# mehta-lab/VisCy

Measured on AMD Instinct MI355X. Metric: training patches/sec (Z=5, 256x256, 1->2ch UNeXt2), higher is better.
Workload: dtype bf16; 1 GPU; UNeXt2 2.5D convnextv2_tiny Z=5 256x256 1->2ch, fwd+MixedLoss(0.5,0,0.5)+bwd+AdamW; per_gpu_batch=512, global_batch=512, parallelism=dp1

## Files before the change

include/vsx.h:

```cpp
#ifndef VSX_H
#define VSX_H
#include <stddef.h>
#include <stdint.h>

#ifdef __cplusplus
extern "C" {
#endif

typedef void* vsx_stream_t;

#define VSX_F32 0
#define VSX_BF16 1

int32_t vsx_version(void);
const char* vsx_last_error(void);
const char* vsx_last_kernel(void);
int32_t vsx_set_flag(const char* name, int32_t value);
int32_t vsx_get_flag(const char* name);
int32_t vsx_det_workspace(float* ws, int64_t floats);
int32_t vsx_det_scope(int32_t on);
int32_t vsx_det_active(void);

#define VSX_A_ROWS 0
#define VSX_A_PATCH2 1
// ... 281 lines not shown
#define VSX_WTASK_REDUCE_ROWS 6
#define VSX_WTASK_MAX 40
typedef struct VsxWTask {
  int32_t kind, dtype, i0, i1, i2, i3;
  const void* p0;
  void* p1;
  void* p2;
  const void* p3;
  const void* p4;
  const void* p5;
  const void* p6;
  const void* p7;
} VsxWTask;
int32_t vsx_weight_tasks(const VsxWTask* tasks, int32_t n, vsx_stream_t stream);

int32_t vsx_prep_head_dgrad(const float* W, void* dst, int32_t Cmid, int32_t C3, int32_t Zout, int32_t dtype,
    vsx_stream_t stream);

int32_t vsx_stem_im2col(const float* x, void* P, const float* sub, const float* div, int32_t B, int32_t Cin,
    int32_t Z, int32_t H, int32_t W, int32_t kz, int32_t ky, int32_t kx, int32_t dtype, vsx_stream_t stream);
int32_t vsx_stem_im2col_ld(const float* x, void* P, const float* sub, const float* div, int32_t B, int32_t Cin, int32_t Z,
    int32_t H, int32_t W, int32_t kz, int32_t ky, int32_t kx, int32_t ldp, int32_t dtype, vsx_stream_t stream);
int32_t vsx_pad_cols(const void* src, void* dst, int32_t R, int32_t K, int32_t Kp, int32_t dtype, vsx_stream_t stream);

int32_t vsx_im2col3x3(const void* x, void* col, int32_t B, int32_t H, int32_t W, int32_t C, int32_t dtype, vsx_stream_t stream);
int32_t vsx_col2im3x3(const void* dcol, void* dx, int32_t B, int32_t H, int32_t W, int32_t C, int32_t dtype, vsx_stream_t stream);

int32_t vsx_pixel_shuffle_cat_fwd(const void* low, const void* skip, void* out, int32_t B, int32_t h,
    int32_t w, int32_t c, int32_t cs, int32_t dtype, vsx_stream_t stream);

int32_t vsx_pixel_shuffle_cat_bwd(const void* dcat, void* dlow, void* dskip, int32_t B, int32_t h, int32_t w,
    int32_t c, int32_t cs, int32_t dtype, vsx_stream_t stream);

int32_t vsx_head_shuffle_fwd(const void* dec, void* hin, int32_t B, int32_t h, int32_t w, int32_t C3,
    int32_t D, int32_t pool, int32_t dtype, vsx_stream_t stream);

int32_t vsx_head_shuffle_bwd(const void* dhin, void* ddec, int32_t B, int32_t h, int32_t w, int32_t C3,
    int32_t D, int32_t pool, int32_t dtype, vsx_stream_t stream);

int32_t vsx_normalize(const float* x, float* y, const float* sub, const float* div, int32_t B, int64_t per_sample,
    vsx_stream_t stream);

int32_t vsx_minmax_norm(const float* x, float* y, const float* lo, const float* hi, int32_t B, int64_t per_sample,
    vsx_stream_t stream);

int32_t vsx_sample_minmax(const float* x, float* mn, float* mx, int32_t B, int64_t per_sample, vsx_stream_t stream);

int32_t vsx_intensity_aug(const float* x, float* y, const float* mn, const float* mx, const float* gamma,
    const float* factor, const float* noise, const float* nstd, float nmean, int32_t invert, int32_t B, int64_t per_sample,
    vsx_stream_t stream);
int32_t vsx_sample_moments(const float* x, double* sums, int32_t B, int64_t per_sample, vsx_stream_t stream);

int32_t vsx_blend_in(const float* oldp, const float* newp, float* out, const float* fz, int32_t Z, int64_t plane,
    int64_t total, vsx_stream_t stream);

int32_t vsx_crop_weights(const float* w, float* wpool, float* tmp, int32_t B, int32_t CZ, int32_t Y, int32_t X,
    int32_t cy, int32_t cx, vsx_stream_t stream);
int32_t vsx_sample_index(const float* wpool, const float* u, int32_t* idx, int32_t B, int64_t n, vsx_stream_t stream);
int32_t vsx_crop3d(const float* x, float* y, const int32_t* starts, int32_t B, int32_t C, int32_t Z, int32_t Y, int32_t X,
    int32_t cz, int32_t cy, int32_t cx, vsx_stream_t stream);

int32_t vsx_warp_affine3d(const float* x, float* y, const float* Minv, int32_t B, int32_t C, int32_t D, int32_t H,
    int32_t W, int32_t mode, vsx_stream_t stream);
int32_t vsx_warp_affine3d_roi(const float* x, float* y, const float* Minv, int32_t B, int32_t C, int32_t D, int32_t H,
    int32_t W, int32_t z0, int32_t y0, int32_t x0, int32_t Do, int32_t Ho, int32_t Wo, int32_t mode, vsx_stream_t stream);

// ... 31 lines not shown
```

viscy_amd/_lib.py:

```python

from __future__ import annotations

import ctypes as C
import os

import torch

_HERE = os.path.dirname(os.path.abspath(__file__))
LIB_PATH = os.environ.get("VSX_LIB", os.path.join(_HERE, "libvsx.so"))

VSX_F32, VSX_BF16 = 0, 1
A_ROWS, A_PATCH2, A_CONV3 = 0, 1, 2
PRO_NONE, PRO_GRN = 0, 1
EPI_NONE, EPI_BIAS, EPI_BIAS_GELU_SQ, EPI_BIAS_RES, EPI_DZ, EPI_BIAS_STATS, EPI_LN_BWD = 0, 1, 2, 3, 4, 5, 6
LOSS_SLOTS, LOSS_SLOT_STRIDE = 64, 32

_I32, _F32, _P, _I64 = C.c_int32, C.c_float, C.c_void_p, C.c_int64


class VsxGemm(C.Structure):
    _fields_ = [
        ("A", _P), ("B", _P), ("C", _P),
        ("M", _I32), ("N", _I32), ("K", _I32),
        ("lda", _I32), ("ldb", _I32), ("ldc", _I32),
# ... 27 lines not shown


WTASK_PREP, WTASK_TRANSPOSE, WTASK_MATVEC, WTASK_MLP_PACK, WTASK_UNPREP, WTASK_MATVEC_T, WTASK_REDUCE_ROWS = 0, 1, 2, 3, 4, 5, 6

_SIGS = {
    "vsx_version": (_I32, []),
    "vsx_weight_tasks": (_I32, [_P, _I32, _P]),
    "vsx_last_error": (C.c_char_p, []),
    "vsx_last_kernel": (C.c_char_p, []),
    "vsx_set_flag": (_I32, [C.c_char_p, _I32]),
    "vsx_get_flag": (_I32, [C.c_char_p]),
    "vsx_det_workspace": (_I32, [_P, _I64]),
    "vsx_det_scope": (_I32, [_I32]),
    "vsx_det_active": (_I32, []),
    "vsx_gemm_nt": (_I32, [C.POINTER(VsxGemm), _I32, _P]),
    "vsx_gemm_tn": (_I32, [C.POINTER(VsxGemm), _I32, _P]),
    "vsx_gemm_plan": (_I32, [_I32, C.POINTER(VsxGemm), _I32, C.POINTER(VsxGemmPlan)]),
    "vsx_gemm_nt_ln_bwd_supported": (_I32, [_I64, _I32, _I32, _I32]),
    "vsx_ln_fwd": (_I32, [_P, _P, _P, _P, _P, _P, _I32, _I32, _F32, _I32, _P]),
    "vsx_ln_bwd": (_I32, [_P, _P, _P, _P, _P, _P, _P, _P, _P, _I32, _I32, _I32, _P]),
    "vsx_grn_scale": (_I32, [_P, _P, _P, _I32, _I32, _F32, _P]),
    "vsx_grn_bwd_stats": (_I32, [_P, _P, _P, _P, _P, _P, _P, _P, _I32, _I32, _F32, _P]),
    "vsx_grn_gelu_bwd": (_I32, [_P, _P, _P, _P, _P, _P, _I32, _I32, _I32, _I32, _I32, _P]),
    "vsx_dwconv7_fwd": (_I32, [_P, _P, _P, _P, _P, _I32, _I32, _I32, _I32, _I32, _P]),
    "vsx_dwconv7_bwd_data": (_I32, [_P, _P, _P, _P, _I32, _I32, _I32, _I32, _I32, _P]),
    "vsx_dwconv7_bwd_weight": (_I32, [_P, _P, _P, _P, _P, _I32, _I32, _I32, _I32, _I32, _I32, _P]),
    "vsx_stem_im2col": (_I32, [_P, _P, _P, _P, _I32, _I32, _I32, _I32, _I32, _I32, _I32, _I32, _I32, _P]),
    "vsx_stem_im2col_ld": (_I32, [_P, _P, _P, _P, _I32, _I32, _I32, _I32, _I32, _I32, _I32, _I32, _I32, _I32, _P]),
    "vsx_pad_cols": (_I32, [_P, _P, _I32, _I32, _I32, _I32, _P]),
    "vsx_im2col3x3": (_I32, [_P, _P, _I32, _I32, _I32, _I32, _I32, _P]),
    "vsx_col2im3x3": (_I32, [_P, _P, _I32, _I32, _I32, _I32, _I32, _P]),
    "vsx_pixel_shuffle_cat_fwd": (_I32, [_P, _P, _P, _I32, _I32, _I32, _I32, _I32, _I32, _P]),
    "vsx_pixel_shuffle_cat_bwd": (_I32, [_P, _P, _P, _I32, _I32, _I32, _I32, _I32, _I32, _P]),
    "vsx_head_shuffle_fwd": (_I32, [_P, _P, _I32, _I32, _I32, _I32, _I32, _I32, _I32, _P]),
    "vsx_head_shuffle_bwd": (_I32, [_P, _P, _I32, _I32, _I32, _I32, _I32, _I32, _I32, _P]),
    "vsx_head_out_fwd": (_I32, [_P] * 7 + [_I32] * 6 + [_F32, _I32, _P]),
    "vsx_head_out_bwd1": (_I32, [_P] * 11 + [_I32] * 6 + [_F32, _I32, _P]),
    "vsx_head_out_bwd1_wgrad": (_I32, [_P] * 13 + [_I32] * 6 + [_F32, _I32, _P]),
    "vsx_head_out_bwd2": (_I32, [_P] * 9 + [_I32] * 6 + [_F32, _I32, _P]),
    "vsx_loss_pool": (_I32, [_P] * 7 + [_I32] * 3 + [_P]),
    "vsx_ssim_scale_fwd": (_I32, [_P] * 5 + [_I32] * 5 + [_P]),
    "vsx_ssim_scale_bwd": (_I32, [_P] * 7 + [_I32] * 5 + [_F32, _F32, _P, _I32, _P]),
    "vsx_loss_finalize": (_I32, [_P] * 5 + [_F32, _I32, _I32, _I32, _F32, _F32, _F32, _P, _P, _P, _P, _P]),
    "vsx_ssim_scale_fwd_dmu": (_I32, [_P] * 6 + [_I32] * 6 + [_P]),
    "vsx_ssim_scale_bwd_in": (_I32, [_P] * 6 + [_I32] * 5 + [_F32, _F32, _P, _I32, _I32, _P]),
    "vsx_loss_tmax": (_I32, [_P, _I64, _P, _P]),
    "vsx_ssim_scale_fwd_fused": (_I32, [_P] * 11 + [_I32] * 6 + [_P]),
    "vsx_adamw": (_I32, [_P, _P, _P, _P, _P, _I64, _P]),
    "vsx_adamw_advance": (_I32, [_P, _P, _P, _P]),
    "vsx_fill_f32": (_I32, [_P, _I64, _F32, _P]),
    "vsx_mlp_supported": (_I32, [_I32, _I32, _I64, _I32]),
    "vsx_mlp_mode_supported": (_I32, [_I32, _I32, _I64, _I32, _I32]),
    "vsx_mlp_det_floats": (_I64, [_I32, _I32, _I64, _I32]),
    "vsx_mlp_image_bytes": (_I64, [_I32]),
    "vsx_mlp_pack": (_I32, [_P, _P, _P, _I32, _P]),
    "vsx_mlp_fwd": (_I32, [_P] * 11 + [_I64, _I32, _I32, _I32, _I32, _P]),
    "vsx_mlp_fc1": (_I32, [_P] * 7 + [_I64, _I32, _I32, _I32, _P]),
    "vsx_mlp_fwd_ln": (_I32, [_P, _F32] + [_P] * 10 + [_I64, _I32, _I32, _I32, _I32, _P]),
    "vsx_mlp_fc1_ln": (_I32, [_P, _F32] + [_P] * 9 + [_I64, _I32, _I32, _I32, _P]),
    "vsx_grn_q_reduce": (_I32, [_P] * 10 + [_I64, _I32, _I32, _I32, _P]),
    "vsx_grn_q_reduce_ws_floats": (_I64, [_I32, _I32]),
    "vsx_mlp_bwd_stats": (_I32, [_P] * 5 + [_I64, _I32, _I32, _I32, _P]),
    "vsx_mlp_bwd_dh": (_I32, [_P] * 7 + [_I64, _P, _P, _I64, _I32, _I32, _I32, _P]),
    "vsx_mlp_rows_per_workgroup": (_I32, [_I32, _I32, _I64]),
    "vsx_mlp_bwd_dh_re": (_I32, [_P] * 9 + [_I64, _P, _P, _I64, _I32, _I32, _I32, _P]),
    "vsx_mlp_bwd_dh_ln": (_I32, [_P] * 11 + [_I64, _P, _P, _I64, _I32, _I32, _I32, _P]),
# ... 124 lines not shown
```

viscy_amd/csrc/norm.hip:

```cpp
#include "vsx_common.h"
#include "wtasks.h"
#include "../../include/vsx.h"

template <typename T, int G, int CPL>
__global__ __launch_bounds__(256) void ln_fwd_kernel(const T* __restrict__ x, T* __restrict__ y,
                                                     float* __restrict__ mean_out, float* __restrict__ rstd_out,
                                                     const float* __restrict__ gamma, const float* __restrict__ beta,
                                                     int rows, int C, float eps, int iters, int nt) {
  constexpr int VN = VT<T>::N;
  constexpr int R = CPL == 1 ? 4 : (CPL == 2 ? 2 : 1);
  constexpr int RPI = 256 / G;
  const int nch = C / VN;
  const int gl = threadIdx.x % G;
  float gam[CPL][VN], bet[CPL][VN];
#pragma unroll
  for (int i = 0; i < CPL; ++i) {
    const int c = gl + i * G;
#pragma unroll
    for (int j = 0; j < VN; ++j) {
      gam[i][j] = (gamma && c < nch) ? gamma[c * VN + j] : 1.f;
      bet[i][j] = (gamma && c < nch) ? beta[c * VN + j] : 0.f;
    }
  }
  for (int it = 0; it < iters; ++it) {
// ... 235 lines not shown
  if (nch <= 192) LN_CASE(64, 3);
  if (nch <= 256) LN_CASE(64, 4);
#undef LN_CASE
  vsx_set_error("layernorm: C=%d too wide (max %d)", C, 256 * VT<T>::N);
  return 1;
}

extern "C" int32_t vsx_ln_fwd(const void* x, void* y, float* mean, float* rstd, const float* gamma, const float* beta,
                              int32_t rows, int32_t C, float eps, int32_t dtype, vsx_stream_t stream) {
  int vn = dtype == VSX_BF16 ? 8 : 4;
  VSX_CHECK(rows > 0 && C > 0 && C % vn == 0, "vsx_ln_fwd: rows=%d C=%d (C must be a multiple of %d)", rows, C, vn);
  VSX_CHECK(x && y && rstd, "vsx_ln_fwd: null pointer");
  VSX_CHECK((gamma == nullptr) == (beta == nullptr), "vsx_ln_fwd: gamma and beta must both be set or both NULL");
  hipStream_t s = (hipStream_t)stream;
  return dtype == VSX_BF16
             ? ln_dispatch<bf16_t>(true, x, nullptr, y, mean, rstd, gamma, beta, nullptr, nullptr, nullptr, rows, C, eps, s)
             : ln_dispatch<float>(true, x, nullptr, y, mean, rstd, gamma, beta, nullptr, nullptr, nullptr, rows, C, eps, s);
}

extern "C" int32_t vsx_ln_bwd(const void* dy, const void* x, const float* mean, const float* rstd, const float* gamma,
                              const void* add, void* dx, float* dgamma, float* dbeta, int32_t rows, int32_t C,
                              int32_t dtype, vsx_stream_t stream) {
  int vn = dtype == VSX_BF16 ? 8 : 4;
  VSX_CHECK(rows > 0 && C > 0 && C % vn == 0, "vsx_ln_bwd: rows=%d C=%d (C must be a multiple of %d)", rows, C, vn);
  VSX_CHECK(dy && x && rstd && dx, "vsx_ln_bwd: null pointer");
  VSX_CHECK((dgamma == nullptr) == (dbeta == nullptr), "vsx_ln_bwd: dgamma and dbeta must both be set or both NULL");
  hipStream_t s = (hipStream_t)stream;
  return dtype == VSX_BF16 ? ln_dispatch<bf16_t>(false, dy, x, dx, (float*)mean, (float*)rstd, gamma, nullptr, add,
                                                 dgamma, dbeta, rows, C, 0.f, s)
                           : ln_dispatch<float>(false, dy, x, dx, (float*)mean, (float*)rstd, gamma, nullptr, add,
                                                dgamma, dbeta, rows, C, 0.f, s);
}

__global__ __launch_bounds__(256) void grn_scale_kernel(const float* __restrict__ colsq, const float* __restrict__ gamma,
                                                        float* __restrict__ s, int N, float eps) {
  __shared__ float part[4];
  const int b = blockIdx.x;
  float acc = 0.f;
  for (int n = threadIdx.x; n < N; n += 256) acc += sqrtf(colsq[(size_t)b * N + n]);
  acc = wave_sum(acc);
  if ((threadIdx.x & 63) == 0) part[threadIdx.x >> 6] = acc;
  __syncthreads();
  const float m = (part[0] + part[1] + part[2] + part[3]) / (float)N;
  for (int n = threadIdx.x; n < N; n += 256)
    s[(size_t)b * N + n] = 1.f + gamma[n] * sqrtf(colsq[(size_t)b * N + n]) / (m + eps);
}

__global__ __launch_bounds__(256) void grn_bwd_stats_kernel(const float* __restrict__ colsq, const float* __restrict__ P,
                                                            const float* __restrict__ gamma, float* __restrict__ t,
                                                            float* __restrict__ wsg, int N, float eps) {
  __shared__ float part[2][4];
  const int b = blockIdx.x;
  float a0 = 0.f, a1 = 0.f;
  for (int n = threadIdx.x; n < N; n += 256) {
    float g = sqrtf(colsq[(size_t)b * N + n]);
    a0 += g;
    a1 += gamma[n] * P[(size_t)b * N + n] * g;
  }
  a0 = wave_sum(a0);
  a1 = wave_sum(a1);
  if ((threadIdx.x & 63) == 0) { part[0][threadIdx.x >> 6] = a0; part[1][threadIdx.x >> 6] = a1; }
  __syncthreads();
  const float m = (part[0][0] + part[0][1] + part[0][2] + part[0][3]) / (float)N;
  const float sdg = part[1][0] + part[1][1] + part[1][2] + part[1][3];
  const float inv = 1.f / (m + eps);
  for (int n = threadIdx.x; n < N; n += 256) {
// ... 278 lines not shown
```

viscy_amd/engine_unext2.py:

```python

from __future__ import annotations

import os
from collections import namedtuple
from typing import NamedTuple

import torch
from torch import Tensor

from . import _lib as L
from . import ops as hip_ops
from .flat import FlatEngine, engine_apply


class _BlockW:

    __slots__ = ("C", "p", "dw_w", "W1f", "W1fT", "b1f", "W2", "W2T", "v1", "fc2_w", "fc2_b", "grn_w", "grn_b", "dp", "img", "img2", "b2f")


class _ProjW:
    __slots__ = ("cin", "cout", "taps", "ln", "conv", "W", "WT")


FWD_UNFUSED, FWD_PAIR, FWD_FC1 = 0, 1, 2
# ... 250 lines not shown
            W["fc0"], W["fc0T"] = o.prep_weight(t.fc0.weight, E, Cf, 1, torch.float32, want=True, want_t=need_bwd)
            W["fc3"], W["fc3T"] = o.prep_weight(t.fc3.weight, P, E, 1, torch.float32, want=True, want_t=need_bwd)
        else:
            for us in m.decoder.decoder_stages:
                st = us.conv
                proj = self._prep_proj(st.downsample[0], st.downsample[1], dt, need_bwd)
                dec.append((proj, [self._prep_block(b, dt, need_bwd) for b in st.blocks]))
            pre = []
            for us in m.decoder.decoder_stages:
                pc = getattr(us, "pre_conv", None)
                if pc is None:
                    pre.append(None)
                else:
                    cpc = pc.weight.shape[0]
                    pre.append((pc, *o.prep_weight(pc.weight, cpc, cpc, 9, dt, want=True, want_t=need_bwd)))
            W["dec_pre"] = pre
        W["dec"] = dec
        if cfg.get("head", "conv") == "conv":
            hc = m.head.conv[0].conv
            cmid, c3 = hc.weight.shape[0], hc.weight.shape[1]
            hdt = self._head_dtype(dt)
            W["head_Wc"], _ = o.prep_weight(hc.weight, cmid, c3, 27, hdt, tapmode=1)
            if need_bwd:
                if hdt == torch.bfloat16 and c3 == 8 and cmid == 32 and cfg["out_stack_depth"] == 5:
                    o.flush()
                    W["head_Wp"] = o.head_conv_dgrad_prep(W["head_Wc"])
                W["head_Wd"] = o.prep_head_dgrad(hc.weight, cmid, c3, cfg["out_stack_depth"], hdt)
        return W

    def _head_dtype(self, dt: torch.dtype) -> torch.dtype:
        if dt == torch.bfloat16 and self.model.head.conv[0].conv.weight.shape[1] % 8:
            return torch.float32
        return dt

    def _plan(self, C, hw, M, B, dt, training: bool) -> _MlpPlan:
        o, flag = self.ops, self._mlp_flag
        ask = training and dt == torch.bfloat16 and flag != 0
        return _plan_mlp(flag, lambda mode: o.mlp_supported(C, hw, M, dt, mode), C, hw, M, B, dt, training,
                         ask and bool(L.lib().vsx_gemm_nt_ln_bwd_supported(M, C, 4 * C, L.dtype_code(dt))),
                         ask and o.tn_grn_stats_ok(M, C, 4 * C, hw, dt))

    def _block_fwd(self, x, w, B, H, Wd, dt, save, rows=None):
        if w.C < 16:
            return self._block_fwd_narrow(x, w, B, H, Wd, save, rows)
        o = self.ops
        C, M = w.C, B * H * Wd
        blk = w.p
        hw = H * Wd
        y = o.dwconv7_fwd(x, w.dw_w, blk.conv_dw.bias, B, H, Wd, C)
        xres = x
        if rows is not None:
            idx, inv, _, Lr = rows
            M, hw = B * Lr, Lr
            y = o.rows_select(y, idx, M, C)
            xres = o.rows_select(x, idx, M, C)
        plan = self._plan(C, hw, M, B, dt, save is not None)
        mean = rstd = None
        if plan.ln_in:
            xh = None
        else:
            xh, _, rstd = o.ln_fwd(y, None, None, M, C, 1e-6, need_mean=False)
            y = None
        colsq = self._za.take(B, 4 * C)
        dpm = None
        if w.dp > 0.0 and self.model.training:
            inj = self._dp_inject
# ... 225 lines not shown
                       a_mode=L.A_PATCH2, gh=ch, gw=cw, cs=cc, epi=L.EPI_BIAS, bias=proj.conv.bias)
                st_sv["proj"] = (cur, xn, mean, rstd)
                cur, cc = nxt, proj.cout
            rows = None
            if masks is not None:
                rows = masks[i]
                cur = o.rows_select(cur, rows[2], B * ch * cw, cc)
            for bw in blocks:
                cur = self._block_fwd(cur, bw, B, ch, cw, dt, st_sv["blocks"] if need_bwd else None, rows)
            feats.append((cur, ch, cw, cc))
            enc_sv.append(st_sv)
        if cfg.get("head") == "embed":
            out = self._embed_tail_fwd(feats[3], B, sv, bn_groups)
            if need_bwd:
                sv["enc"] = enc_sv
                sv["feat_dims"] = [(a, b_, c) for (_, a, b_, c) in feats]
            self._za_need[za_key] = za.used
            return out, sv
        dec_sv = []
        feat, fh, fw, fc = feats[3]
        for k, (proj, blocks) in enumerate(W["dec"]):
            skip, sh, sw_, sc = feats[2 - k]
            assert sh == 2 * fh and sw_ == 2 * fw
            c_up = fc // 4
            pre = W["dec_pre"][k]
            low_in = None
            if pre is not None:
                pc, Wp, _ = pre
                col = o.im2col3x3(feat, B, fh, fw, fc)
                low_in = feat
                feat = torch.empty((B * fh * fw, fc), dtype=dt, device=x.device)
                o.gemm("nt", col, Wp, feat, B * fh * fw, fc, 9 * fc, 9 * fc, 9 * fc, fc, dtype=dt, epi=L.EPI_BIAS, bias=pc.bias)
                del col
            cat = o.pixel_shuffle_cat_fwd(feat, skip, B, fh, fw, c_up, sc)
            fh, fw = sh, sw_
            Mk, ccat = B * fh * fw, c_up + sc
            if proj.cout < 16:
                cur, mean, rstd = o.narrow_proj_fwd(cat, proj.ln.weight, proj.ln.bias, proj.conv.weight, proj.conv.bias, Mk, ccat,
                                                    proj.cout)
                xn = None
            else:
                xn, mean, rstd = o.ln_fwd(cat, proj.ln.weight, proj.ln.bias, Mk, ccat)
                cur = torch.empty((Mk, proj.cout), dtype=dt, device=x.device)
                o.gemm("nt", xn, proj.W, cur, Mk, proj.cout, ccat, ccat, ccat, proj.cout, dtype=dt, epi=L.EPI_BIAS,
                       bias=proj.conv.bias)
            st_sv = {"proj": (cat, xn, mean, rstd, c_up, sc), "blocks": [], "pre_in": low_in}
            for bw in blocks:
                cur = self._block_fwd(cur, bw, B, fh, fw, dt, st_sv["blocks"] if need_bwd else None)
            feat, fc = cur, proj.cout
            dec_sv.append(st_sv)
        if cfg.get("head", "conv") == "shuffle":
            sxy = cfg["stem_kernel"][-1]
            out = o.voxel_shuffle_fwd(feat, B, fh, fw, cfg["out_channels"], cfg["out_stack_depth"], sxy, True)
            if need_bwd:
                sv["enc"], sv["dec"] = enc_sv, dec_sv
                sv["feat_dims"] = [(a, b_, c) for (_, a, b_, c) in feats]
                sv["head"] = (fh, fw)
            self._za_need[za_key] = za.used
            return out, sv
        Zo, D7 = cfg["out_stack_depth"], cfg["out_stack_depth"] + 2
        hc = m.head.conv[0].conv
        cmid, c3 = hc.weight.shape[0], hc.weight.shape[1]
        cout = cfg["out_channels"]
        hdt = self._head_dtype(dt)
        hin = o.head_shuffle_fwd(feat if hdt == dt else feat.float(), B, fh, fw, c3, D7, cfg["head_pool"])
        H2, W2 = 2 * fh, 2 * fw
        Mh = B * H2 * W2
        stats = self._za.take(2, B, cmid)
        direct = o.head_conv_supported(H2, W2, c3, cmid, Zo, hdt)
        if direct:
            U = o.head_conv_fwd(hin, W["head_Wc"], hc.bias, stats[0], stats[1], B, H2, W2, c3, cmid, Zo)
        else:
            U = torch.empty((Mh, Zo * cmid), dtype=hdt, device=x.device)
            o.gemm_z("nt", hin, W["head_Wc"], U, Mh, cmid, 27 * c3, D7 * c3, 27 * c3, Zo * cmid, dtype=hdt,
                     a_mode=L.A_CONV3, gh=H2, gw=W2, cs=3 * c3, nz=Zo, a_coff=[z * c3 for z in range(Zo)],
                     b_off=[0] * Zo, c_coff=[z * cmid for z in range(Zo)], epi=L.EPI_BIAS_STATS, bias=hc.bias,
                     red0=stats[0], red1=stats[1], hw=H2 * W2)
        w2 = m.head.conv[1].weight.view(4 * cout, cmid)
        out = o.head_out_fwd(U, stats[0], stats[1], w2, m.head.conv[1].bias, m.head.conv[0].adn.A.weight, B, H2, W2, Zo,
# ... 122 lines not shown
            za_key = ("bwd", B, H, Wd, sv["masked"])
            self._za = za = _ZeroArena(dev, self._za_need.get(za_key, 0), self.ops)
            if cfg.get("head") == "embed":
                d = self._embed_tail_bwd(sv, dout[0], dout[1], dt, B)
            elif cfg.get("head", "conv") == "shuffle":
                fh, fw = sv["head"]
                sxy = cfg["stem_kernel"][-1]
                vs = o.voxel_shuffle_bwd
                if (cfg["out_channels"] * cfg["out_stack_depth"] * sxy * sxy) % (8 if dt == torch.bfloat16 else 4):
                    vs = o.narrow_voxel_shuffle_bwd
                d = vs(dout.contiguous().float(), B, fh, fw, cfg["out_channels"], cfg["out_stack_depth"], sxy, True, dt)
            else:
                hdt = self._head_dtype(dt)
                d = self._head_conv_bwd(sv, dout, hdt, B, dev)
                if hdt != dt:
                    d = d.to(dt)
            dskips = {}
            for k in (2, 1, 0) if cfg.get("head") != "embed" else ():
                proj, blocks = W["dec"][k]
                st_sv = sv["dec"][k]
                cat, xn, mean, rstd, c_up, sc = st_sv["proj"]
                _, sh, sw_, _ = (None, *sv["feat_dims"][2 - k])
                Mk, ccat = B * sh * sw_, c_up + sc
                for bw, bsv in zip(reversed(blocks), reversed(st_sv["blocks"])):
                    d = self._block_bwd(d, bw, bsv, B, sh, sw_, dt)
                if proj.cout < 16:
                    dxn = o.narrow_proj_bwd(d, cat, mean, rstd, proj.ln.weight, proj.ln.bias, proj.conv.weight, g(proj.conv.weight),
                                            g(proj.conv.bias), Mk, ccat, proj.cout)
                else:
                    o.gemm("tn", xn, d, g(proj.conv.weight), Mk, proj.cout, ccat, ccat, proj.cout, ccat, dtype=dt,
                           colsum=g(proj.conv.bias))
                    dxn = torch.empty((Mk, ccat), dtype=dt, device=dev)
                    o.gemm("nt", d, proj.WT, dxn, Mk, ccat, proj.cout, proj.cout, proj.cout, ccat, dtype=dt)
                dcat = o.ln_bwd(dxn, cat, mean, rstd, proj.ln.weight, None, g(proj.ln.weight), g(proj.ln.bias), Mk, ccat)
                del dxn
                d, dskips[2 - k] = o.pixel_shuffle_cat_bwd(dcat, B, sh // 2, sw_ // 2, c_up, sc)
                del dcat
                pre = W["dec_pre"][k]
                if pre is not None:
                    pc, _, WpT = pre
                    lh, lw, cpc = sh // 2, sw_ // 2, 4 * c_up
                    Ml = B * lh * lw
                    col = o.im2col3x3(st_sv["pre_in"], B, lh, lw, cpc)
                    dWp = self._za.take(cpc, 9 * cpc)
                    o.gemm("tn", col, d, dWp, Ml, cpc, 9 * cpc, 9 * cpc, cpc, 9 * cpc, dtype=dt, colsum=g(pc.bias))
                    o.unprep_grad(dWp, g(pc.weight), cpc, cpc, 9)
                    del col
                    dcol = torch.empty((Ml, 9 * cpc), dtype=dt, device=dev)
                    o.gemm("nt", d, WpT, dcol, Ml, 9 * cpc, cpc, cpc, cpc, 9 * cpc, dtype=dt)
                    d = o.col2im3x3(dcol, B, lh, lw, cpc)
                    del dcol
            yield from self._segment_end(0)
            if self.encoder_frozen():
                self._za_need[za_key] = za.used
                yield from self._segment_end(1)
                yield from self._segment_end(2)
                return
            for i in (3, 2, 1, 0):
                proj, blocks = W["enc"][i]
                st_sv = sv["enc"][i]
                ch, cw, cc = sv["feat_dims"][i]
                for bw, bsv in zip(reversed(blocks), reversed(st_sv["blocks"])):
                    d = self._block_bwd(d, bw, bsv, B, ch, cw, dt)
                if proj is not None:
                    prev, xn, mean, rstd = st_sv["proj"]
                    cin = proj.cin
                    Mo = B * ch * cw
                    dWg = self._za.take(proj.cout, 4 * cin)
                    o.gemm("tn", xn, d, dWg, Mo, proj.cout, 4 * cin, cin, proj.cout, 4 * cin, dtype=dt, a_mode=L.A_PATCH2,
                           gh=ch, gw=cw, cs=cin, colsum=g(proj.conv.bias))
# ... 46 lines not shown
```

viscy_amd/ops.py:

```python

from __future__ import annotations

import contextlib
import ctypes as C
import os
import threading
from typing import Sequence

import torch
from torch import Tensor

from . import _lib as L
from ._lib import VsxGemm, VsxGemmPlan, check, dtype_code, lib, ptr, stream


class Scratch:

    def __init__(self, alloc=None):
        self._alloc = alloc or (lambda floats, dev: torch.empty(floats, dtype=torch.float32, device=dev))
        self._tls = threading.local()
        self.held: list = []

    def take(self, dev, floats: int):
        arenas = getattr(self._tls, "arenas", None)
# ... 229 lines not shown
    col = torch.empty((B * H * W, 9 * Cc), dtype=x.dtype, device=x.device)
    check(lib().vsx_im2col3x3(ptr(x), ptr(col), B, H, W, Cc, dtype_code(x.dtype), stream()), "im2col3x3")
    return col


def col2im3x3(dcol: Tensor, B: int, H: int, W: int, Cc: int) -> Tensor:
    dx = torch.empty((B * H * W, Cc), dtype=dcol.dtype, device=dcol.device)
    check(lib().vsx_col2im3x3(ptr(dcol), ptr(dx), B, H, W, Cc, dtype_code(dcol.dtype), stream()), "col2im3x3")
    return dx


def pad_cols(src: Tensor, Kp: int) -> Tensor:
    R, K = src.shape
    dst = torch.empty((R, Kp), dtype=src.dtype, device=src.device)
    check(lib().vsx_pad_cols(ptr(src), ptr(dst), R, K, Kp, dtype_code(src.dtype), stream()), "pad_cols")
    return dst


def pixel_shuffle_cat_fwd(low: Tensor, skip: Tensor | None, B: int, h: int, w: int, c: int, cs: int) -> Tensor:
    out = torch.empty((B * 4 * h * w, c + cs), dtype=low.dtype, device=low.device)
    check(lib().vsx_pixel_shuffle_cat_fwd(ptr(low), ptr(skip), ptr(out), B, h, w, c, cs, dtype_code(low.dtype), stream()),
          "pixel_shuffle_cat_fwd")
    return out


def pixel_shuffle_cat_bwd(dcat: Tensor, B: int, h: int, w: int, c: int, cs: int):
    dlow = torch.empty((B * h * w, 4 * c), dtype=dcat.dtype, device=dcat.device)
    dskip = torch.empty((B * 4 * h * w, cs), dtype=dcat.dtype, device=dcat.device) if cs else None
    check(lib().vsx_pixel_shuffle_cat_bwd(ptr(dcat), ptr(dlow), ptr(dskip), B, h, w, c, cs, dtype_code(dcat.dtype),
                                          stream()), "pixel_shuffle_cat_bwd")
    return dlow, dskip


def head_shuffle_fwd(dec: Tensor, B: int, h: int, w: int, C3: int, D: int, pool: bool) -> Tensor:
    hin = torch.empty((B * 4 * h * w, C3 * D), dtype=dec.dtype, device=dec.device)
    check(lib().vsx_head_shuffle_fwd(ptr(dec), ptr(hin), B, h, w, C3, D, int(pool), dtype_code(dec.dtype), stream()),
          "head_shuffle_fwd")
    return hin


def head_shuffle_bwd(dhin: Tensor, B: int, h: int, w: int, C3: int, D: int, pool: bool) -> Tensor:
    ddec = torch.empty((B * h * w, 4 * C3 * D), dtype=dhin.dtype, device=dhin.device)
    check(lib().vsx_head_shuffle_bwd(ptr(dhin), ptr(ddec), B, h, w, C3, D, int(pool), dtype_code(dhin.dtype), stream()),
          "head_shuffle_bwd")
    return ddec


def head_out_fwd(U, ssum, ssq, w2, b2, alpha, B, H2, W2, Z, Cmid, Cout, eps=1e-5) -> Tensor:
    out = torch.empty((B, Cout, Z, 2 * H2, 2 * W2), dtype=torch.float32, device=U.device)
    check(lib().vsx_head_out_fwd(ptr(U), ptr(ssum), ptr(ssq), ptr(w2), ptr(b2), ptr(alpha), ptr(out), B, H2, W2, Z, Cmid,
                                 Cout, eps, dtype_code(U.dtype), stream()), "head_out_fwd")
    return out


def head_out_bwd1(U, ssum, ssq, w2, alpha, dout, S1, S2, dalpha, B, H2, W2, Z, Cmid, Cout, eps=1e-5):
    M5 = B * H2 * W2 * Z
    act = torch.empty((M5, Cmid), dtype=U.dtype, device=U.device)
    dv = torch.empty((M5, 4 * Cout), dtype=U.dtype, device=U.device)
    check(lib().vsx_head_out_bwd1(ptr(U), ptr(ssum), ptr(ssq), ptr(w2), ptr(alpha), ptr(dout), ptr(act), ptr(dv), ptr(S1),
                                  ptr(S2), ptr(dalpha), B, H2, W2, Z, Cmid, Cout, eps, dtype_code(U.dtype), stream()),
          "head_out_bwd1")
    return act, dv


def head_out_bwd1_wgrad(U, ssum, ssq, w2, alpha, dout, S1, S2, dalpha, dW2, db2, B, H2, W2, Z, Cmid, Cout, eps=1e-5) -> Tensor:
    M5 = B * H2 * W2 * Z
# ... 639 lines not shown
```

Before: 5616 patches/s.

## Fuse decoder pixel-shuffle+concat into LayerNorm forward and backward

Adds HIP kernels that read the low-resolution feature and the skip tensor directly, de-interleaving the pixel-shuffle quads in registers, and apply LayerNorm without materialising the concatenated tensor. The matching backward computes the LN gradient and scatters it straight into dlow/dskip, removing the intermediate dcat buffer and one kernel pass each way. The decoder keeps low/skip instead of cat for backward. It adds complexity, and the eps default (1e-6) must match the original LN.

```diff
diff --git a/include/vsx.h b/include/vsx.h
--- a/include/vsx.h
+++ b/include/vsx.h
@@ -337,6 +337,14 @@
 int32_t vsx_pixel_shuffle_cat_bwd(const void* dcat, void* dlow, void* dskip, int32_t B, int32_t h, int32_t w,
     int32_t c, int32_t cs, int32_t dtype, vsx_stream_t stream);
 
+int32_t vsx_ps_cat_ln_supported(int32_t c, int32_t cs, int32_t dtype);
+int32_t vsx_ps_cat_ln_fwd(const void* low, const void* skip, void* xn, float* mean, float* rstd, const float* gamma,
+    const float* beta, int32_t B, int32_t h, int32_t w, int32_t c, int32_t cs, float eps, int32_t dtype, vsx_stream_t stream);
+
+int32_t vsx_ln_bwd_ps_cat(const void* dxn, const void* low, const void* skip, const float* mean, const float* rstd,
+    const float* gamma, void* dlow, void* dskip, float* dgamma, float* dbeta, int32_t B, int32_t h, int32_t w, int32_t c,
+    int32_t cs, int32_t dtype, vsx_stream_t stream);
+
 int32_t vsx_head_shuffle_fwd(const void* dec, void* hin, int32_t B, int32_t h, int32_t w, int32_t C3,
     int32_t D, int32_t pool, int32_t dtype, vsx_stream_t stream);
 
diff --git a/viscy_amd/_lib.py b/viscy_amd/_lib.py
--- a/viscy_amd/_lib.py
+++ b/viscy_amd/_lib.py
@@ -83,6 +83,9 @@
     "vsx_col2im3x3": (_I32, [_P, _P, _I32, _I32, _I32, _I32, _I32, _P]),
     "vsx_pixel_shuffle_cat_fwd": (_I32, [_P, _P, _P, _I32, _I32, _I32, _I32, _I32, _I32, _P]),
     "vsx_pixel_shuffle_cat_bwd": (_I32, [_P, _P, _P, _I32, _I32, _I32, _I32, _I32, _I32, _P]),
+    "vsx_ps_cat_ln_supported": (_I32, [_I32, _I32, _I32]),
+    "vsx_ps_cat_ln_fwd": (_I32, [_P] * 7 + [_I32] * 5 + [_F32, _I32, _P]),
+    "vsx_ln_bwd_ps_cat": (_I32, [_P] * 10 + [_I32] * 6 + [_P]),
     "vsx_head_shuffle_fwd": (_I32, [_P, _P, _I32, _I32, _I32, _I32, _I32, _I32, _I32, _P]),
     "vsx_head_shuffle_bwd": (_I32, [_P, _P, _I32, _I32, _I32, _I32, _I32, _I32, _I32, _P]),
     "vsx_head_out_fwd": (_I32, [_P] * 7 + [_I32] * 6 + [_F32, _I32, _P]),
diff --git a/viscy_amd/csrc/norm.hip b/viscy_amd/csrc/norm.hip
--- a/viscy_amd/csrc/norm.hip
+++ b/viscy_amd/csrc/norm.hip
@@ -291,6 +291,368 @@
                                                 dgamma, dbeta, rows, C, 0.f, s);
 }
 
+template <typename T>
+struct QuadGeom {
+  const T* low;
+  const T* skip;
+  int h, w, c, cs;
+};
+
+__device__ __forceinline__ size_t quad_pix00(int q, int h, int w) {
+  const int x = q % w;
+  const int r = q / w;
+  const int y = r % h;
+  const int b = r / h;
+  return ((size_t)b * (2 * h) + 2 * y) * (size_t)(2 * w) + 2 * x;
+}
+
+__device__ __forceinline__ void quad_deinterleave(const float4 (&lo)[4], float4 (&rows)[4]) {
+  rows[0] = make_float4(lo[0].x, lo[1].x, lo[2].x, lo[3].x);
+  rows[1] = make_float4(lo[0].y, lo[1].y, lo[2].y, lo[3].y);
+  rows[2] = make_float4(lo[0].z, lo[1].z, lo[2].z, lo[3].z);
+  rows[3] = make_float4(lo[0].w, lo[1].w, lo[2].w, lo[3].w);
+}
+__device__ __forceinline__ void quad_interleave(const float4 (&rows)[4], float4 (&lo)[4]) {
+  lo[0] = make_float4(rows[0].x, rows[1].x, rows[2].x, rows[3].x);
+  lo[1] = make_float4(rows[0].y, rows[1].y, rows[2].y, rows[3].y);
+  lo[2] = make_float4(rows[0].z, rows[1].z, rows[2].z, rows[3].z);
+  lo[3] = make_float4(rows[0].w, rows[1].w, rows[2].w, rows[3].w);
+}
+__device__ __forceinline__ uint32_t lo16_pair(uint32_t a, uint32_t b) { return (a & 0xffffu) | (b << 16); }
+__device__ __forceinline__ uint32_t hi16_pair(uint32_t a, uint32_t b) { return (a >> 16) | (b & 0xffff0000u); }
+__device__ __forceinline__ void quad_deinterleave(const uint4 (&lo)[4], uint4 (&rows)[4]) {
+  rows[0] = make_uint4(lo16_pair(lo[0].x, lo[0].z), lo16_pair(lo[1].x, lo[1].z), lo16_pair(lo[2].x, lo[2].z), lo16_pair(lo[3].x, lo[3].z));
+  rows[1] = make_uint4(hi16_pair(lo[0].x, lo[0].z), hi16_pair(lo[1].x, lo[1].z), hi16_pair(lo[2].x, lo[2].z), hi16_pair(lo[3].x, lo[3].z));
+  rows[2] = make_uint4(lo16_pair(lo[0].y, lo[0].w), lo16_pair(lo[1].y, lo[1].w), lo16_pair(lo[2].y, lo[2].w), lo16_pair(lo[3].y, lo[3].w));
+  rows[3] = make_uint4(hi16_pair(lo[0].y, lo[0].w), hi16_pair(lo[1].y, lo[1].w), hi16_pair(lo[2].y, lo[2].w), hi16_pair(lo[3].y, lo[3].w));
+}
+__device__ __forceinline__ uint4 quad_interleave_word(uint32_t r0, uint32_t r1, uint32_t r2, uint32_t r3) {
+  return make_uint4(lo16_pair(r0, r1), lo16_pair(r2, r3), hi16_pair(r0, r1), hi16_pair(r2, r3));
+}
+__device__ __forceinline__ void quad_interleave(const uint4 (&rows)[4], uint4 (&lo)[4]) {
+  lo[0] = quad_interleave_word(rows[0].x, rows[1].x, rows[2].x, rows[3].x);
+  lo[1] = quad_interleave_word(rows[0].y, rows[1].y, rows[2].y, rows[3].y);
+  lo[2] = quad_interleave_word(rows[0].z, rows[1].z, rows[2].z, rows[3].z);
+  lo[3] = quad_interleave_word(rows[0].w, rows[1].w, rows[2].w, rows[3].w);
+}
+
+template <typename T, bool NT>
+__device__ __forceinline__ void quad_load(const QuadGeom<T>& g, int q, size_t pix00, int cv, typename VT<T>::vec (&rows)[4]) {
+  constexpr int VN = VT<T>::N;
+  typedef typename VT<T>::vec vec;
+  const int ng = g.c / VN;
+  if (cv < ng) {
+    vec lo[4];
+    const T* lp = g.low + (size_t)q * (4 * g.c) + (size_t)cv * (4 * VN);
+#pragma unroll
+    for (int v = 0; v < 4; ++v) lo[v] = ldvec_stream<T>(lp + v * VN, NT);
+    quad_deinterleave(lo, rows);
+  } else {
+#pragma unroll
+    for (int s = 0; s < 4; ++s)
+      rows[s] = ldvec_stream<T>(g.skip + (pix00 + (s >> 1) * (2 * g.w) + (s & 1)) * g.cs + (size_t)(cv - ng) * VN, NT);
+  }
+}
+
+template <typename T, int G, int CPL, bool NT>
+__global__ __launch_bounds__(256) void ps_cat_ln_fwd_kernel(QuadGeom<T> geo, T* __restrict__ y, float* __restrict__ mean_out,
+                                                            float* __restrict__ rstd_out, const float* __restrict__ gamma,
+                                                            const float* __restrict__ beta, int quads, float eps, int iters) {
+  constexpr int VN = VT<T>::N;
+  typedef typename VT<T>::vec vec;
+  constexpr int QPI = 256 / G;
+  const int C = geo.c + geo.cs;
+  const int nch = C / VN;
+  const int gl = threadIdx.x % G;
+  float gam[CPL][VN], bet[CPL][VN];
+#pragma unroll
+  for (int i = 0; i < CPL; ++i) {
+    const int c = gl + i * G;
+#pragma unroll
+    for (int j = 0; j < VN; ++j) {
+      gam[i][j] = c < nch ? gamma[c * VN + j] : 1.f;
+      bet[i][j] = c < nch ? beta[c * VN + j] : 0.f;
+    }
+  }
+  for (int it = 0; it < iters; ++it) {
+    const int q = (it * gridDim.x + blockIdx.x) * QPI + threadIdx.x / G;
+    const bool live = q < quads;
+    const int ql = live ? q : quads - 1;
+    const size_t pix00 = quad_pix00(ql, geo.h, geo.w);
+    vec xr[CPL][4];
+#pragma unroll
+    for (int i = 0; i < CPL; ++i) {
+      const int c = gl + i * G;
+      if (c < nch) quad_load<T, NT>(geo, ql, pix00, c, xr[i]);
+    }
+#pragma unroll
+    for (int s4 = 0; s4 < 4; ++s4) {
+      const size_t row = pix00 + (s4 >> 1) * (2 * geo.w) + (s4 & 1);
+      float v[CPL][VN];
+#pragma unroll
+      for (int i = 0; i < CPL; ++i) {
+        if (gl + i * G < nch) {
+          unpack<T>(xr[i][s4], v[i]);
+        } else {
+#pragma unroll
+          for (int j = 0; j < VN; ++j) v[i][j] = 0.f;
+        }
+      }
+      const float x0 = __shfl(v[0][0], (threadIdx.x & 63) / G * G, 64);
+      float s = 0.f, sq = 0.f;
+#pragma unroll
+      for (int i = 0; i < CPL; ++i) {
+        if (gl + i * G < nch) {
+#pragma unroll
+          for (int j = 0; j < VN; ++j) {
+            const float d = v[i][j] - x0;
+            s += d;
+            sq = fmaf(d, d, sq);
+          }
+        }
+      }
+      s = group_sum<G>(s) / (float)C;
+      sq = group_sum<G>(sq) / (float)C;
+      const float mean = x0 + s;
+      const float rstd = rsqrtf(fmaxf(sq - s * s, 0.f) + eps);
+      if (live) {
+        T* yr = y + row * C;
+#pragma unroll
+        for (int i = 0; i < CPL; ++i) {
+          const int c = gl + i * G;
+          if (c < nch) {
+            float o[VN];
+#pragma unroll
+            for (int j = 0; j < VN; ++j) {
+              const float xh = (v[i][j] - mean) * rstd;
+              o[j] = fmaf(xh, gam[i][j], bet[i][j]);
+            }
+            stvec<T>(yr + c * VN, pack<T>(o));
+          }
+        }
+        if (gl == 0) {
+          mean_out[row] = mean;
+          rstd_out[row] = rstd;
+        }
+      }
+    }
+  }
+}
+
+template <typename T, int G, int CPL, bool NT>
+__global__ __launch_bounds__(256) void ps_cat_ln_bwd_kernel(const T* __restrict__ dy, QuadGeom<T> geo,
+                                                            const float* __restrict__ mean, const float* __restrict__ rstd,
+                                                            const float* __restrict__ gamma, T* __restrict__ dlow,
+                                                            T* __restrict__ dskip, float* __restrict__ dgamma,
+                                                            float* __restrict__ dbeta, int quads, int iters) {
+  constexpr int VN = VT<T>::N;
+  typedef typename VT<T>::vec vec;
+  constexpr int QPI = 256 / G;
+  extern __shared__ float red[];
+  const int C = geo.c + geo.cs;
+  const int nch = C / VN, ng = geo.c / VN;
+  const int gl = threadIdx.x % G;
+  if (dgamma) {
+    for (int i = threadIdx.x; i < 2 * C; i += 256) red[i] = 0.f;
+    __syncthreads();
+  }
+  float dg[CPL][VN], db[CPL][VN], gam[CPL][VN];
+#pragma unroll
+  for (int i = 0; i < CPL; ++i) {
+    const int c = gl + i * G;
+#pragma unroll
+    for (int j = 0; j < VN; ++j) {
+      dg[i][j] = 0.f;
+      db[i][j] = 0.f;
+      gam[i][j] = c < nch ? gamma[c * VN + j] : 1.f;
+    }
+  }
+  for (int it = 0; it < iters; ++it) {
+    const int q = (it * gridDim.x + blockIdx.x) * QPI + threadIdx.x / G;
+    const bool live = q < quads;
+    const int ql = live ? q : 0;
+    const size_t pix00 = quad_pix00(ql, geo.h, geo.w);
+    vec xr[CPL][4], dr[CPL][4];
+    float mu4[4], rs4[4];
+#pragma unroll
+    for (int s4 = 0; s4 < 4; ++s4) {
+      const size_t row = pix00 + (s4 >> 1) * (2 * geo.w) + (s4 & 1);
+      mu4[s4] = live ? mean[row] : 0.f;
+      rs4[s4] = live ? rstd[row] : 0.f;
+    }
+#pragma unroll
+    for (int i = 0; i < CPL; ++i) {
+      const int c = gl + i * G;
+      if (c < nch) {
+        quad_load<T, NT>(geo, ql, pix00, c, xr[i]);
+#pragma unroll
+        for (int s4 = 0; s4 < 4; ++s4)
+          dr[i][s4] = ldvec_stream<T>(dy + (pix00 + (s4 >> 1) * (2 * geo.w) + (s4 & 1)) * C + c * VN, NT);
+      }
+    }
+#pragma unroll
+    for (int s4 = 0; s4 < 4; ++s4) {
+      const float mu = mu4[s4], rs = rs4[s4];
+      float xh[CPL][VN], g[CPL][VN];
+      float s1 = 0.f, s2 = 0.f;
+#pragma unroll
+      for (int i = 0; i < CPL; ++i) {
+        const int c = gl + i * G;
+        if (c < nch && live) {
+          float xv[VN], dv[VN];
+          unpack<T>(xr[i][s4], xv);
+          unpack<T>(dr[i][s4], dv);
+#pragma unroll
+          for (int j = 0; j < VN; ++j) {
+            xh[i][j] = (xv[j] - mu) * rs;
+            g[i][j] = dv[j] * gam[i][j];
+            dg[i][j] += dv[j] * xh[i][j];
+            db[i][j] += dv[j];
+            s1 += g[i][j];
+            s2 += g[i][j] * xh[i][j];
+          }
+        } else {
+#pragma unroll
+          for (int j = 0; j < VN; ++j) { xh[i][j] = 0.f; g[i][j] = 0.f; }
+        }
+      }
+      s1 = group_sum<G>(s1) / (float)C;
+      s2 = group_sum<G>(s2) / (float)C;
+#pragma unroll
+      for (int i = 0; i < CPL; ++i) {
+        float o[VN];
+#pragma unroll
+        for (int j = 0; j < VN; ++j) o[j] = rs * (g[i][j] - s1 - xh[i][j] * s2);
+        dr[i][s4] = pack<T>(o);
+      }
+      __builtin_amdgcn_sched_barrier(0);
+    }
+    if (live) {
+#pragma unroll
+      for (int i = 0; i < CPL; ++i) {
+        const int c = gl + i * G;
+        if (c < ng) {
+          vec lo[4];
+          quad_interleave(dr[i], lo);
+          T* lp = dlow + (size_t)ql * (4 * geo.c) + (size_t)c * (4 * VN);
+#pragma unroll
+          for (int v = 0; v < 4; ++v) stvec<T>(lp + v * VN, lo[v]);
+        } else if (c < nch) {
+#pragma unroll
+          for (int s4 = 0; s4 < 4; ++s4)
+            stvec<T>(dskip + (pix00 + (s4 >> 1) * (2 * geo.w) + (s4 & 1)) * geo.cs + (size_t)(c - ng) * VN, dr[i][s4]);
+        }
+      }
+    }
+  }
+  if (dgamma) {
+#pragma unroll
+    for (int i = 0; i < CPL; ++i) {
+      const int c = gl + i * G;
+      if (c < nch) {
+#pragma unroll
+        for (int j = 0; j < VN; ++j) {
+          atomicAdd(&red[c * VN + j], dg[i][j]);
+          atomicAdd(&red[C + c * VN + j], db[i][j]);
+        }
+      }
+    }
+    __syncthreads();
+    for (int i = threadIdx.x; i < C; i += 256) {
+      atomicAdd(dgamma + i, red[i]);
+      atomicAdd(dbeta + i, red[C + i]);
+    }
+  }
+}
+
+struct PsCatLnArgs {
+  const void *dxn, *low, *skip, *gamma, *beta;
+  void *xn, *mean, *rstd, *dlow, *dskip, *dgamma, *dbeta;
+  int B, h, w, c, cs;
+  float eps;
+};
+
+template <typename T, int G, int CPL, bool NT>
+static int ps_cat_ln_launch(bool fwd, const PsCatLnArgs& a, hipStream_t s) {
+  constexpr int QPI = 256 / G;
+  const int quads = a.B * a.h * a.w;
+  const QuadGeom<T> geo = {(const T*)a.low, (const T*)a.skip, a.h, a.w, a.c, a.cs};
+  if (fwd) {
+    const int fcap = g_vsx_ln_fblk >= 8 ? g_vsx_ln_fblk / 8 : 1;
+    int iters = vsx_cdiv(quads, QPI * fcap);
+    if (iters < 1) iters = 1;
+    hipLaunchKernelGGL((ps_cat_ln_fwd_kernel<T, G, CPL, NT>), dim3(vsx_cdiv(quads, QPI * iters)), dim3(256), 0, s, geo, (T*)a.xn,
+                       (float*)a.mean, (float*)a.rstd, (const float*)a.gamma, (const float*)a.beta, quads, a.eps, iters);
+  } else {
+    int iters = vsx_cdiv(quads, QPI * g_vsx_ln_ablk);
+    if (iters < 1) iters = 1;
+    const size_t sh = a.dgamma ? 2 * (size_t)(a.c + a.cs) * sizeof(float) : 0;
+    hipLaunchKernelGGL((ps_cat_ln_bwd_kernel<T, G, CPL, NT>), dim3(vsx_cdiv(quads, QPI * iters)), dim3(256), sh, s,
+                       (const T*)a.dxn, geo, (const float*)a.mean, (const float*)a.rstd, (const float*)a.gamma, (T*)a.dlow,
+                       (T*)a.dskip, (float*)a.dgamma, (float*)a.dbeta, quads, iters);
+  }
+  VSX_LAUNCH_CHECK();
+  return 0;
+}
+
+template <typename T>
+static int ps_cat_ln_dispatch(bool fwd, const PsCatLnArgs& a, hipStream_t s) {
+  const int nch = (a.c + a.cs) / VT<T>::N;
+  const bool nt = g_vsx_ln_stream & (fwd ? 2 : 1);
+#define PCL_CASE(G, CPL) return nt ? ps_cat_ln_launch<T, G, CPL, true>(fwd, a, s) : ps_cat_ln_launch<T, G, CPL, false>(fwd, a, s)
+  if (g_vsx_ln_pack && !fwd) {
+    if (nch == 24) PCL_CASE(8, 3);
+    if (nch == 48) PCL_CASE(16, 3);
+  }
+  if (nch <= 4) PCL_CASE(4, 1);
+  if (nch <= 8) PCL_CASE(8, 1);
+  if (nch <= 16) PCL_CASE(16, 1);
+  if (nch <= 32) PCL_CASE(32, 1);
+  if (nch <= 64) PCL_CASE(64, 1);
+  if (nch <= 128) PCL_CASE(64, 2);
+  if (nch <= 192) PCL_CASE(64, 3);
+  PCL_CASE(64, 4);
+#undef PCL_CASE
+}
+
+extern "C" int32_t vsx_ps_cat_ln_supported(int32_t c, int32_t cs, int32_t dtype) {
+  if (dtype != VSX_BF16 && dtype != VSX_F32) return 0;
+  const int vn = dtype == VSX_BF16 ? 8 : 4;
+  return c > 0 && cs > 0 && c % vn == 0 && cs % vn == 0 && (c + cs) / vn <= 256;
+}
+
+extern "C" int32_t vsx_ps_cat_ln_fwd(const void* low, const void* skip, void* xn, float* mean, float* rstd, const float* gamma,
+                                     const float* beta, int32_t B, int32_t h, int32_t w, int32_t c, int32_t cs, float eps,
+                                     int32_t dtype, vsx_stream_t stream) {
+  const int vn = dtype == VSX_BF16 ? 8 : 4;
+  VSX_CHECK(B > 0 && h > 0 && w > 0 && (int64_t)B * h * w <= INT32_MAX / 4, "vsx_ps_cat_ln_fwd: bad arguments");
+  VSX_CHECK(vsx_ps_cat_ln_supported(c, cs, dtype),
+            "vsx_ps_cat_ln_fwd: c=%d cs=%d (both must be positive multiples of %d, c+cs at most %d)", c, cs, vn, 256 * vn);
+  VSX_CHECK(low && skip && xn && mean && rstd && gamma && beta, "vsx_ps_cat_ln_fwd: null pointer");
+  PsCatLnArgs a = {};
+  a.low = low; a.skip = skip; a.xn = xn; a.mean = mean; a.rstd = rstd; a.gamma = gamma; a.beta = beta;
+  a.B = B; a.h = h; a.w = w; a.c = c; a.cs = cs; a.eps = eps;
+  return dtype == VSX_BF16 ? ps_cat_ln_dispatch<bf16_t>(true, a, (hipStream_t)stream)
+                           : ps_cat_ln_dispatch<float>(true, a, (hipStream_t)stream);
+}
+
+extern "C" int32_t vsx_ln_bwd_ps_cat(const void* dxn, const void* low, const void* skip, const float* mean, const float* rstd,
+                                     const float* gamma, void* dlow, void* dskip, float* dgamma, float* dbeta, int32_t B,
+                                     int32_t h, int32_t w, int32_t c, int32_t cs, int32_t dtype, vsx_stream_t stream) {
+  const int vn = dtype == VSX_BF16 ? 8 : 4;
+  VSX_CHECK(B > 0 && h > 0 && w > 0 && (int64_t)B * h * w <= INT32_MAX / 4, "vsx_ln_bwd_ps_cat: bad arguments");
+  VSX_CHECK(vsx_ps_cat_ln_supported(c, cs, dtype),
+            "vsx_ln_bwd_ps_cat: c=%d cs=%d (both must be positive multiples of %d, c+cs at most %d)", c, cs, vn, 256 * vn);
+  VSX_CHECK(dxn && low && skip && mean && rstd && gamma && dlow && dskip, "vsx_ln_bwd_ps_cat: null pointer");
+  VSX_CHECK((dgamma == nullptr) == (dbeta == nullptr), "vsx_ln_bwd_ps_cat: dgamma and dbeta must both be set or both NULL");
+  PsCatLnArgs a = {};
+  a.dxn = dxn; a.low = low; a.skip = skip; a.mean = (void*)mean; a.rstd = (void*)rstd; a.gamma = gamma;
+  a.dlow = dlow; a.dskip = dskip; a.dgamma = dgamma; a.dbeta = dbeta;
+  a.B = B; a.h = h; a.w = w; a.c = c; a.cs = cs;
+  return dtype == VSX_BF16 ? ps_cat_ln_dispatch<bf16_t>(false, a, (hipStream_t)stream)
+                           : ps_cat_ln_dispatch<float>(false, a, (hipStream_t)stream);
+}
+
 __global__ __launch_bounds__(256) void grn_scale_kernel(const float* __restrict__ colsq, const float* __restrict__ gamma,
                                                         float* __restrict__ s, int N, float eps) {
   __shared__ float part[4];
diff --git a/viscy_amd/engine_unext2.py b/viscy_amd/engine_unext2.py
--- a/viscy_amd/engine_unext2.py
+++ b/viscy_amd/engine_unext2.py
@@ -306,6 +306,12 @@
         if dt == torch.bfloat16 and self.model.head.conv[0].conv.weight.shape[1] % 8:
             return torch.float32
         return dt
+
+    dec_entry_fused = True
+
+    def _dec_entry_fused(self, c_up: int, sc: int, cout: int, dt: torch.dtype) -> bool:
+        return (self._hip and self.dec_entry_fused and cout >= 16
+                and bool(L.lib().vsx_ps_cat_ln_supported(c_up, sc, L.dtype_code(dt))))
 
     def _plan(self, C, hw, M, B, dt, training: bool) -> _MlpPlan:
         o, flag = self.ops, self._mlp_flag
@@ -597,19 +603,24 @@
                 feat = torch.empty((B * fh * fw, fc), dtype=dt, device=x.device)
                 o.gemm("nt", col, Wp, feat, B * fh * fw, fc, 9 * fc, 9 * fc, 9 * fc, fc, dtype=dt, epi=L.EPI_BIAS, bias=pc.bias)
                 del col
-            cat = o.pixel_shuffle_cat_fwd(feat, skip, B, fh, fw, c_up, sc)
-            fh, fw = sh, sw_
-            Mk, ccat = B * fh * fw, c_up + sc
-            if proj.cout < 16:
+            fused = self._dec_entry_fused(c_up, sc, proj.cout, dt)
+            cat = None if fused else o.pixel_shuffle_cat_fwd(feat, skip, B, fh, fw, c_up, sc)
+            Mk, ccat = B * sh * sw_, c_up + sc
+            if fused:
+                xn, mean, rstd = o.ps_cat_ln_fwd(feat, skip, proj.ln.weight, proj.ln.bias, B, fh, fw, c_up, sc)
+            elif proj.cout < 16:
                 cur, mean, rstd = o.narrow_proj_fwd(cat, proj.ln.weight, proj.ln.bias, proj.conv.weight, proj.conv.bias, Mk, ccat,
                                                     proj.cout)
                 xn = None
             else:
                 xn, mean, rstd = o.ln_fwd(cat, proj.ln.weight, proj.ln.bias, Mk, ccat)
+            if xn is not None:
                 cur = torch.empty((Mk, proj.cout), dtype=dt, device=x.device)
                 o.gemm("nt", xn, proj.W, cur, Mk, proj.cout, ccat, ccat, ccat, proj.cout, dtype=dt, epi=L.EPI_BIAS,
                        bias=proj.conv.bias)
-            st_sv = {"proj": (cat, xn, mean, rstd, c_up, sc), "blocks": [], "pre_in": low_in}
+            fh, fw = sh, sw_
+            st_sv = {"proj": (cat, xn, mean, rstd, c_up, sc), "low_skip": (feat, skip) if fused and need_bwd else None,
+                     "blocks": [], "pre_in": low_in}
             for bw in blocks:
                 cur = self._block_fwd(cur, bw, B, fh, fw, dt, st_sv["blocks"] if need_bwd else None)
             feat, fc = cur, proj.cout
@@ -798,10 +809,16 @@
                            colsum=g(proj.conv.bias))
                     dxn = torch.empty((Mk, ccat), dtype=dt, device=dev)
                     o.gemm("nt", d, proj.WT, dxn, Mk, ccat, proj.cout, proj.cout, proj.cout, ccat, dtype=dt)
-                dcat = o.ln_bwd(dxn, cat, mean, rstd, proj.ln.weight, None, g(proj.ln.weight), g(proj.ln.bias), Mk, ccat)
-                del dxn
-                d, dskips[2 - k] = o.pixel_shuffle_cat_bwd(dcat, B, sh // 2, sw_ // 2, c_up, sc)
-                del dcat
+                if st_sv["low_skip"] is not None:
+                    low, skip = st_sv["low_skip"]
+                    d, dskips[2 - k] = o.ln_bwd_ps_cat(dxn, low, skip, mean, rstd, proj.ln.weight, g(proj.ln.weight),
+                                                       g(proj.ln.bias), B, sh // 2, sw_ // 2, c_up, sc)
+                    del dxn, low, skip
+                else:
+                    dcat = o.ln_bwd(dxn, cat, mean, rstd, proj.ln.weight, None, g(proj.ln.weight), g(proj.ln.bias), Mk, ccat)
+                    del dxn
+                    d, dskips[2 - k] = o.pixel_shuffle_cat_bwd(dcat, B, sh // 2, sw_ // 2, c_up, sc)
+                    del dcat
                 pre = W["dec_pre"][k]
                 if pre is not None:
                     pc, _, WpT = pre
diff --git a/viscy_amd/ops.py b/viscy_amd/ops.py
--- a/viscy_amd/ops.py
+++ b/viscy_amd/ops.py
@@ -285,6 +285,30 @@
     return dlow, dskip
 
 
+def ps_cat_ln_supported(c: int, cs: int, dtype: torch.dtype) -> bool:
+    return bool(lib().vsx_ps_cat_ln_supported(c, cs, dtype_code(dtype)))
+
+
+def ps_cat_ln_fwd(low: Tensor, skip: Tensor, gamma: Tensor, beta: Tensor, B: int, h: int, w: int, c: int, cs: int,
+                  eps: float = 1e-6):
+    rows = B * 4 * h * w
+    xn = torch.empty((rows, c + cs), dtype=low.dtype, device=low.device)
+    mean = torch.empty(rows, dtype=torch.float32, device=low.device)
+    rstd = torch.empty(rows, dtype=torch.float32, device=low.device)
+    check(lib().vsx_ps_cat_ln_fwd(ptr(low), ptr(skip), ptr(xn), ptr(mean), ptr(rstd), ptr(gamma), ptr(beta), B, h, w, c, cs, eps,
+                                  dtype_code(low.dtype), stream()), "ps_cat_ln_fwd")
+    return xn, mean, rstd
+
+
+def ln_bwd_ps_cat(dxn: Tensor, low: Tensor, skip: Tensor, mean: Tensor, rstd: Tensor, gamma: Tensor, dgamma: Tensor | None,
+                  dbeta: Tensor | None, B: int, h: int, w: int, c: int, cs: int):
+    dlow = torch.empty((B * h * w, 4 * c), dtype=dxn.dtype, device=dxn.device)
+    dskip = torch.empty((B * 4 * h * w, cs), dtype=dxn.dtype, device=dxn.device)
+    check(lib().vsx_ln_bwd_ps_cat(ptr(dxn), ptr(low), ptr(skip), ptr(mean), ptr(rstd), ptr(gamma), ptr(dlow), ptr(dskip),
+                                  ptr(dgamma), ptr(dbeta), B, h, w, c, cs, dtype_code(dxn.dtype), stream()), "ln_bwd_ps_cat")
+    return dlow, dskip
+
+
 def head_shuffle_fwd(dec: Tensor, B: int, h: int, w: int, C3: int, D: int, pool: bool) -> Tensor:
     hin = torch.empty((B * 4 * h * w, C3 * D), dtype=dec.dtype, device=dec.device)
     check(lib().vsx_head_shuffle_fwd(ptr(dec), ptr(hin), B, h, w, C3, D, int(pool), dtype_code(dec.dtype), stream()),
```

After: 5669 patches/s, median of 6. Within noise of the previous version (+1.0%).
